# openai/gym

Hardware: AMD Instinct MI355X
Metric: env-steps/sec at num_envs=2^20, CartPole-v1 (higher is better)
Workload: dtype f64

## Files before the change

gym_amd/csrc/mxv_device.hpp:

```cpp
#pragma once
#include <hip/hip_runtime.h>
#include <stdint.h>

#include "../../include/mxv.h"
#include "../../include/mxv_diag.h"
#include "mxv_divide.hpp"

#define MXV_XFN __device__ inline
#define MXV_XCONST __device__ const
#define MXV_XCOLD __device__ __noinline__ inline
#include "mxv_exact.hpp"

namespace mxv {

struct EnvParams {
    double p[MXV_MAX_PARAMS];
};

enum { PM_BROADCAST = 0, PM_DEFAULT = 1, PM_PER_ENV = 2 };
template <int DEF>
struct Par {
    const EnvParams &P;
    const double *pe;
    int64_t n, e;
// ... 122 lines not shown
    return philox4x32_10_vkey(c, (uint32_t)seed, (uint32_t)(seed >> 32));
}

__device__ __forceinline__ uint32_t step_noise_word(uint64_t seed, uint64_t t) {
    U4 c;
    c.x = (uint32_t)t;
    c.y = (uint32_t)(t >> 32);
    c.z = 0;
    c.w = (kStreamStepNoise << 28);
    return philox4x32_10_vkey(c, (uint32_t)seed, (uint32_t)(seed >> 32)).x;
}

__device__ __forceinline__ double div_by_const(double x, double c, double rc) {
    const double q0 = x * rc;
    const double r = __fma_rn(-c, q0, x);
    return __fma_rn(r, rc, q0);
}
template <int DEF, bool FINITE = true>
__device__ __forceinline__ double div_par(double x, double c) {
    if constexpr (DEF == PM_DEFAULT && FINITE)
        return div_by_const(x, c, 1.0 / c);
    else if constexpr (DEF == PM_DEFAULT)
        return __builtin_amdgcn_div_fixup(div_by_const(x, c, 1.0 / c), c, x);
    else
        return x / c;
}

template <int ENV>
constexpr int fma3_for() {
    return ((ENV == MXV_PENDULUM || ENV == MXV_MOUNTAINCAR_CONT) ? 1 : 0) | ((ENV == MXV_ACROBOT || ENV == MXV_PENDULUM) ? 2 : 0);
}

template <int F3>
__device__ __forceinline__ double fma_coef(double a, double b, double k) {
    if constexpr ((F3 & 1) != 0) {
        double r;
        asm("v_fma_f64 %0, %1, %2, %3" : "=v"(r) : "v"(a), "v"(b), "v"(k));
        return r;
    } else {
        return __fma_rn(a, b, k);
    }
}

template <int F3 = 0>
__device__ __forceinline__ void sincos_kernel(double x, double *sn, double *cs) {
    const double z = x * x;
    double r = fma_coef<F3>(z, 1.58969099521155010221e-10, -2.50507602534068634195e-08);
    r = fma_coef<F3>(z, r, 2.75573137070700676789e-06);
    r = fma_coef<F3>(z, r, -1.98412698298579493134e-04);
    r = fma_coef<F3>(z, r, 8.33333333332248946124e-03);
    r = fma_coef<F3>(z, r, -1.66666666666666324348e-01);
    *sn = __fma_rn(x * z, r, x);
    double c = fma_coef<F3>(z, -1.13596475577881948265e-11, 2.08757232129817482790e-09);
    c = fma_coef<F3>(z, c, -2.75573143513906633035e-07);
    c = fma_coef<F3>(z, c, 2.48015872894767294178e-05);
    c = fma_coef<F3>(z, c, -1.38888888888741095749e-03);
    c = fma_coef<F3>(z, c, 4.16666666666666019037e-02);
    c = __fma_rn(z, c, -0.5);
    *cs = __fma_rn(z, c, 1.0);
}

template <int F3 = 0>
__device__ __forceinline__ void sincos_medium(double x, double *sn, double *cs) {
    const double k = rint(x * 6.36619772367581382433e-01);
    double r = __fma_rn(-k, 1.5707963267341256, x);
    r = __fma_rn(-k, 6.077100506303966e-11, r);
    r = __fma_rn(-k, 2.0222662487959506e-21, r);
    double s, c;
    sincos_kernel<F3>(r, &s, &c);
    const uint32_t q = (uint32_t)(int)k;
    const bool swap = (q & 1u) != 0u;
    const double ss = swap ? c : s, cc = swap ? s : c;
    if constexpr ((F3 & 2) != 0) {
        *sn = __hiloint2double((int)xor_masked(__double2hiint(ss), q << 30, 0x80000000u), __double2loint(ss));
        *cs = __hiloint2double((int)xor_masked(__double2hiint(cc), (q + 1u) << 30, 0x80000000u), __double2loint(cc));
    } else {
        *sn = __hiloint2double(__double2hiint(ss) ^ (int)((q & 2u) << 30), __double2loint(ss));
        *cs = __hiloint2double(__double2hiint(cc) ^ (int)(((q + 1u) & 2u) << 30), __double2loint(cc));
    }
}
template <bool GUARD = true, int F3 = 0>
__device__ __forceinline__ void mx_sincos(double x, double *sn, double *cs) {
    if constexpr (!GUARD) {
        sincos_medium<F3>(x, sn, cs);
    } else if (fabs(x) < 256.0) {
        sincos_medium<F3>(x, sn, cs);
        if (x == 0.0) *sn = x;
    } else {
        sincos(x, sn, cs);
    }
}
template <bool GUARD = true, int F3 = 0>
__device__ __forceinline__ double mx_cos(double x) {
    double s, c;
    mx_sincos<GUARD, F3>(x, &s, &c);
    return c;
}
template <bool GUARD = true, int F3 = 0>
__device__ __forceinline__ double mx_sin(double x) {
    double s, c;
    mx_sincos<GUARD, F3>(x, &s, &c);
    return s;
}

__device__ __forceinline__ void sincos_small_or_general(double x, double *sn, double *cs) {
    if (fabs(x) <= 0.78539816339744830962) {
        sincos_kernel(x, sn, cs);
        if (x == 0.0) *sn = x;
    } else {
        mx_sincos(x, sn, cs);
    }
}

__device__ __forceinline__ double nan_through(double x, double r) {
    const bool nan = x != x;
    return __hiloint2double(nan ? __double2hiint(x) : __double2hiint(r), nan ? __double2loint(x) : __double2loint(r));
}
__device__ __forceinline__ double clamp_range(double x, double lo, double hi) {
    return nan_through(x, __builtin_fmin(__builtin_fmax(x, lo), hi));
}
__device__ __forceinline__ float clamp_range(float x, float lo, float hi) {
    float r;
    asm("v_maximum3_f32 %0, %1, %2, %2" : "=v"(r) : "v"(x), "v"(lo));
    asm("v_minimum3_f32 %0, %1, %2, %2" : "=v"(r) : "v"(r), "v"(hi));
    return r;
}
__device__ __forceinline__ double clamp_range_hi_first(double x, double lo, double hi) {
    return nan_through(x, __builtin_fmax(__builtin_fmin(x, hi), lo));
}
__device__ __forceinline__ float clamp_range_hi_first(float x, float lo, float hi) {
    float r;
    asm("v_minimum3_f32 %0, %1, %2, %2" : "=v"(r) : "v"(x), "v"(hi));
    asm("v_maximum3_f32 %0, %1, %2, %2" : "=v"(r) : "v"(r), "v"(lo));
    return r;
}

__device__ __forceinline__ double fmod_const(double a, double b, double inv_b) {
    const double aa = fabs(a);
    if (!(aa < 1048576.0 * b)) return fmod(a, b);
    const double q = trunc(aa * inv_b);
    double r = __fma_rn(-q, b, aa);
    if (r < 0.0) r += b;
    else if (r >= b) r -= b;
    return copysign(r, a);
}

template <int ENV>
struct Env;

template <>
struct Env<MXV_CARTPOLE> {
    static constexpr int S = 4, O = 4, NA = 2;
    static constexpr int AUX = 0;
    template <bool GUARD = true>
    __device__ __forceinline__ static void prime(const double *s, double *aux) {}
    template <int DEF, bool SAFE = true, int EPL = 0>
    __device__ __forceinline__ static bool step(const Par<DEF> &P, double *s, double *, bool, int ai, float, double &reward,
                                                float *obs) {
        const double gravity = P.get(0, 9.8), masspole = P.get(2, 0.1), total_mass = P.get(3, 0.1 + 1.0);
        const double length = P.get(4, 0.5), polemass_length = P.get(5, 0.1 * 0.5), force_mag = P.get(6, 10.0);
        const double tau = P.get(7, 0.02), theta_thr = P.get(8, 12 * 2 * kPi / 360), x_thr = P.get(9, 2.4);
        const bool semi_implicit = P.get(10, 0.0) != 0.0;
        double x = s[0], x_dot = s[1], theta = s[2], theta_dot = s[3];
        const double force = (ai == 1) ? force_mag : -force_mag;
        double sintheta, costheta;
        if constexpr (DEF == PM_DEFAULT && !SAFE)
            sincos_kernel<((fma3_for<MXV_CARTPOLE>() & 1) || EPL == 1) ? 1 : 0>(theta, &sintheta, &costheta);
        else
            sincos_small_or_general(theta, &sintheta, &costheta);
        const double temp = div_par<DEF, !SAFE>(force + polemass_length * (theta_dot * theta_dot) * sintheta, total_mass);
        const double ta_num = gravity * sintheta - costheta * temp;
        const double ta_den = length * (4.0 / 3.0 - div_par<DEF, !SAFE>(masspole * (costheta * costheta), total_mass));
        double thetaacc;
        if constexpr (DEF == PM_DEFAULT && !SAFE)
            thetaacc = div_with_rcp(ta_num, ta_den, refined_rcp(ta_den));
        else
            thetaacc = ta_num / ta_den;
        const double xacc = temp - div_par<DEF, !SAFE>(polemass_length * thetaacc * costheta, total_mass);
        if (!semi_implicit) {
            x = x + tau * x_dot;
            x_dot = x_dot + tau * xacc;
            theta = theta + tau * theta_dot;
            theta_dot = theta_dot + tau * thetaacc;
        } else {
            x_dot = x_dot + tau * xacc;
            x = x + tau * x_dot;
            theta_dot = theta_dot + tau * thetaacc;
            theta = theta + tau * theta_dot;
        }
        s[0] = x; s[1] = x_dot; s[2] = theta; s[3] = theta_dot;
        reward = 1.0;
        obs[0] = (float)x; obs[1] = (float)x_dot; obs[2] = (float)theta; obs[3] = (float)theta_dot;
        return (x < -x_thr) || (x > x_thr) || (theta < -theta_thr) || (theta > theta_thr);
    }
    template <bool GUARD = true>
    __device__ __forceinline__ static void observe(const double *s, float *obs, double * = nullptr) {
        obs[0] = (float)s[0]; obs[1] = (float)s[1]; obs[2] = (float)s[2]; obs[3] = (float)s[3];
    }
    __device__ __forceinline__ static void reset(U4 w, double b0, double b1, double *s) {
        s[0] = b0 + (b1 - b0) * u01(w.x);
        s[1] = b0 + (b1 - b0) * u01(w.y);
        s[2] = b0 + (b1 - b0) * u01(w.z);
        s[3] = b0 + (b1 - b0) * u01(w.w);
    }
};

#ifndef MXV_PENDULUM_GLIBC_POWF
#define MXV_PENDULUM_GLIBC_POWF 0
#endif
static __device__ const uint64_t kExp2fTab[32] = {
    0x3ff0000000000000ull, 0x3fefd9b0d3158574ull, 0x3fefb5586cf9890full, 0x3fef9301d0125b51ull,
    0x3fef72b83c7d517bull, 0x3fef54873168b9aaull, 0x3fef387a6e756238ull, 0x3fef1e9df51fdee1ull,
    0x3fef06fe0a31b715ull, 0x3feef1a7373aa9cbull, 0x3feedea64c123422ull, 0x3feece086061892dull,
    0x3feebfdad5362a27ull, 0x3feeb42b569d4f82ull, 0x3feeab07dd485429ull, 0x3feea47eb03a5585ull,
    0x3feea09e667f3bcdull, 0x3fee9f75e8ec5f74ull, 0x3feea11473eb0187ull, 0x3feea589994cce13ull,
    0x3feeace5422aa0dbull, 0x3feeb737b0cdc5e5ull, 0x3feec49182a3f090ull, 0x3feed503b23e255dull,
    0x3feee89f995ad3adull, 0x3feeff76f2fb5e47ull, 0x3fef199bdd85529cull, 0x3fef3720dcef9069ull,
    0x3fef5818dcfba487ull, 0x3fef7c97337b9b5full, 0x3fefa4afa2a490daull, 0x3fefd0765b6e4540ull,
};
static __device__ const double kPowfLog2Tab[16][2] = {
    {0x1.661ec79f8f3bep+0, -0x1.efec65b963019p-2}, {0x1.571ed4aaf883dp+0, -0x1.b0b6832d4fca4p-2},
    {0x1.49539f0f010b0p+0, -0x1.7418b0a1fb77bp-2}, {0x1.3c995b0b80385p+0, -0x1.39de91a6dcf7bp-2},
    {0x1.30d190c8864a5p+0, -0x1.01d9bf3f2b631p-2}, {0x1.25e227b0b8ea0p+0, -0x1.97c1d1b3b7af0p-3},
    {0x1.1bb4a4a1a343fp+0, -0x1.2f9e393af3c9fp-3}, {0x1.12358f08ae5bap+0, -0x1.960cbbf788d5cp-4},
    {0x1.0953f419900a7p+0, -0x1.a6f9db6475fcep-5}, {0x1.0000000000000p+0, 0x0.0p+0},
    {0x1.e608cfd9a47acp-1, 0x1.338ca9f24f53dp-4},  {0x1.ca4b31f026aa0p-1, 0x1.476a9543891bap-3},
    {0x1.b2036576afce6p-1, 0x1.e840b4ac4e4d2p-3},  {0x1.9c2d163a1aa2dp-1, 0x1.40645f0c6651cp-2},
    {0x1.886e6037841edp-1, 0x1.88e9c2c1b9ff8p-2},  {0x1.767dcf5534862p-1, 0x1.ce0a44eb17bccp-2},
};
__device__ __forceinline__ float glibc_powf_square(float x) {
    uint32_t ix = __float_as_uint(x) & 0x7fffffffu;
    if (ix - 0x00800000u >= 0x7f800000u - 0x00800000u) {
        if (ix == 0u || ix >= 0x7f800000u) return x * x;
        ix = __float_as_uint(x * 0x1p23f) & 0x7fffffffu;
        ix -= 23u << 23;
    }
    const uint32_t tmp = ix - 0x3f330000u;
    const uint32_t i = (tmp >> 19) & 15u;
    const uint32_t top = tmp & 0xff800000u;
    const double k = (double)((int32_t)top >> 23);
    const double z = (double)__uint_as_float(ix - top);
    const double invc = kPowfLog2Tab[i][0], logc = kPowfLog2Tab[i][1];
    const double r = z * invc - 1.0;
    const double y0 = logc + k;
    const double r2 = r * r;
    double y = 0x1.27616c9496e0bp-2 * r + -0x1.71969a075c67ap-2;
    const double p = 0x1.ec70a6ca7baddp-2 * r + -0x1.7154748bef6c8p-1;
    const double r4 = r2 * r2;
    double q = 0x1.71547652ab82bp+0 * r + y0;
    q = p * r2 + q;
    y = y * r4 + q;
    const double ylogx = 2.0 * y;
    if (ylogx <= -150.0) return 0.0f;
    if (ylogx > 0x1.fffffffd1d571p+6) return __uint_as_float(0x7f800000u);
    double kd = ylogx + 0x1.8p+47;
    const uint64_t ki = (uint64_t)__double_as_longlong(kd);
    kd -= 0x1.8p+47;
    const double rr = ylogx - kd;
    uint64_t t = kExp2fTab[ki & 31u];
    t += ki << 47;
    const double sc = __longlong_as_double((long long)t);
    const double zz = 0x1.c6af84b912394p-5 * rr + 0x1.ebfce50fac4f3p-3;
    const double rr2 = rr * rr;
    double yy = 0x1.62e42ff0c52d6p-1 * rr + 1.0;
    yy = zz * rr2 + yy;
    yy = yy * sc;
    return (float)yy;
}

__device__ __forceinline__ double np_remainder(double a, double b) {
    double mod = fmod_const(a, b, 1.0 / b);
    if (b == 0.0) return mod;
    if (mod != 0.0) {
        if ((b < 0) != (mod < 0)) mod += b;
    } else {
        mod = copysign(0.0, b);
    }
    return mod;
}
__device__ __forceinline__ double np_remainder_bounded(double a, double b) {
    const double aa = fabs(a);
    const double q = trunc(aa * (1.0 / b));
    double r = __fma_rn(-q, b, aa);
    const double up = r + b, down = r - b;
    r = (r < 0.0) ? up : ((r >= b) ? down : r);
    double mod = copysign(r, a);
    const double lifted = mod + b;
    mod = (mod < 0.0) ? lifted : mod;
    return (mod == 0.0) ? 0.0 : mod;
}

template <>
struct Env<MXV_PENDULUM> {
    static constexpr int S = 2, O = 3, NA = 0;
    static constexpr int AUX = 1;
    template <bool GUARD = true>
    __device__ __forceinline__ static void prime(const double *s, double *aux) { aux[0] = mx_sin<GUARD, fma3_for<MXV_PENDULUM>()>(s[0]); }
    template <bool GUARD = true, int F3 = fma3_for<MXV_PENDULUM>()>
    __device__ __forceinline__ static void observe(const double *s, float *obs, double *aux) {
        double sn, cs;
        mx_sincos<GUARD, F3>(s[0], &sn, &cs);
        obs[0] = (float)cs; obs[1] = (float)sn; obs[2] = (float)s[1];
        aux[0] = sn;
    }
    template <int DEF, bool SAFE = true, int EPL = 0>
    __device__ __forceinline__ static bool step(const Par<DEF> &P, double *s, double *aux, bool, int, float a0,
// ... 296 lines not shown
```

gym_amd/csrc/mxv_kernels.hip:

```cpp
#include <cstdlib>
#include <type_traits>

#include "mxv_host.hpp"
#include "mxv_kernels.hpp"

namespace mxv {

namespace {

__device__ __forceinline__ void raise_error(int32_t *err, int32_t bit) { *reinterpret_cast<volatile int32_t *>(err) = bit; }

typedef float f32x4_t __attribute__((ext_vector_type(4)));
typedef float f32x2_t __attribute__((ext_vector_type(2)));
typedef int i32x4_t __attribute__((ext_vector_type(4)));
typedef int i32x2_t __attribute__((ext_vector_type(2)));
template <bool NT, typename T>
__device__ __forceinline__ void st(T *p, T v) {
    if constexpr (NT) __builtin_nontemporal_store(v, p);
    else *p = v;
}
__device__ __forceinline__ int32_t load_elapsed(const void *p, int32_t el16, int64_t e) {
    return el16 ? (int32_t) static_cast<const uint16_t *>(p)[e] : static_cast<const int32_t *>(p)[e];
}
template <bool NT = false>
// ... 261 lines not shown

        float obs[E][O];
        double rew[E];
        bool term[E], trunc[E], pend[E];
#pragma unroll
        for (int j = 0; j < E; ++j) {
            term[j] = EV::template step<DEF>(P.at(valid[j] ? env_of(j) : 0), s[j], aux[j], el[j] == 0, ai[j], af[j], rew[j], obs[j]);
            el[j] += 1;
            trunc[j] = (a.max_steps > 0) && (el[j] >= a.max_steps);
            pend[j] = autoreset && (term[j] || trunc[j]);
        }
        if (a.ep_acc != nullptr) {
#pragma unroll
            for (int j = 0; j < E; ++j) {
                er[j] = (float)((double)er[j] + rew[j]);
                if (valid[j] && (term[j] || trunc[j])) {
                    if (a.ep_return_out) a.ep_return_out[so + env_of(j)] = er[j];
                    if (a.ep_length_out) a.ep_length_out[so + env_of(j)] = el[j];
                    er[j] = 0.0f;
                }
            }
        }

        while (true) {
            int jsel = -1;
#pragma unroll
            for (int j = E - 1; j >= 0; --j)
                if (pend[j]) jsel = j;
            if (!__any(jsel >= 0)) break;
            if (jsel >= 0) {
                const int64_t e = tile0 + (int64_t)jsel * kBlock + tid;
                bool v = false;
                uint32_t k_reset = 0;
                float cur[O];
#pragma unroll
                for (int j = 0; j < E; ++j)
                    if (j == jsel) {
                        v = valid[j];
                        k_reset = ep[j];
#pragma unroll
                        for (int k = 0; k < O; ++k) cur[k] = obs[j][k];
                    }
                if (a.final_obs != nullptr && v) store_obs<O>(a.final_obs, so + e, cur);
                if constexpr (LAZY_EP) {
                    k_reset = landed(a.episodes[v ? e : 0]);
                    if (v) a.episodes[e] = k_reset + 1;
                }
                const uint64_t seed = a.seeds ? landed(a.seeds[v ? e : 0]) : a.base_seed + a.env0 + (uint64_t)e;
                const U4 w = episode_reset_words(seed, k_reset);
                double ns[S], naux[AUXN];
                float nobs[O];
                EV::reset(w, a.b0, a.b1, ns);
                EV::observe(ns, nobs, naux);
#pragma unroll
                for (int j = 0; j < E; ++j)
                    if (j == jsel) {
#pragma unroll
                        for (int k = 0; k < EV::AUX; ++k) aux[j][k] = naux[k];
#pragma unroll
                        for (int k = 0; k < S; ++k) s[j][k] = ns[k];
#pragma unroll
                        for (int k = 0; k < O; ++k) obs[j][k] = nobs[k];
                        el[j] = 0;
                        if constexpr (!LAZY_EP) ep[j] += 1;
                        pend[j] = false;
                    }
            }
        }

#pragma unroll
        for (int j = 0; j < E; ++j) {
            if (!valid[j]) continue;
            const int64_t e = so + env_of(j);
            store_obs<O, NT>(a.obs, e, obs[j]);
            if (a.reward != nullptr) {
                if (a.flags & MXV_FLAG_REWARD_F32)
                    st<NT>(static_cast<float *>(a.reward) + e, (float)rew[j]);
                else
                    st<NT>(static_cast<double *>(a.reward) + e, rew[j]);
            }
            if (a.terminated != nullptr) st<NT>(a.terminated + e, (uint8_t)(term[j] ? 1 : 0));
            if (a.truncated != nullptr) st<NT>(a.truncated + e, (uint8_t)(trunc[j] ? 1 : 0));
        }
        if constexpr (ENV == MXV_CARTPOLE) {
            if (a.beyond != nullptr) {
#pragma unroll
                for (int j = 0; j < E; ++j)
                    if (valid[j] && term[j]) {
                        uint8_t *mark = a.beyond + env_of(j);
                        if (landed((uint32_t)*mark) == 0u) {
                            *mark = 1;
                        } else if (a.reward != nullptr) {
                            if (a.flags & MXV_FLAG_REWARD_F32)
                                static_cast<float *>(a.reward)[so + env_of(j)] = 0.0f;
                            else
                                static_cast<double *>(a.reward)[so + env_of(j)] = 0.0;
                        }
                    }
            }
        }
    }

#pragma unroll
    for (int j = 0; j < E; ++j) {
        if (!valid[j]) continue;
        const int64_t e = env_of(j);
        if constexpr (HILO) {
            int32_t l[S];
            bool esc = false;
#pragma unroll
            for (int k = 0; k < S; ++k) {
                l[k] = hilo_encode_fast(s[j][k]);
                esc = esc || l[k] == kHiloEscape;
            }
            if (__builtin_expect(__any(esc), 0)) {
#pragma unroll
                for (int k = 0; k < S; ++k)
                    if (l[k] == kHiloEscape) a.state[(int64_t)k * n + e] = s[j][k];
            }
            store_lo<S, NT>(a.lo, e, l);
        } else {
#pragma unroll
            for (int k = 0; k < S; ++k) st<NT>(a.state + (int64_t)k * n + e, s[j][k]);
        }
        store_elapsed<NT>(a.elapsed, a.elapsed16, e, el[j]);
        if (ep[j] != ep_in[j]) a.episodes[e] = ep[j];
        if (a.ep_acc) a.ep_acc[e] = er[j];
    }
    if constexpr (CLOCK) {
        if (tid == 0) {
            const uint32_t ticket = atomicAdd(a.clock_ticket, 1u);
            if (ticket == gridDim.x - 1) {
                *a.clock_ticket = 0u;
                *a.clock_out = t0 - a.t + (uint64_t)a.K;
            }
        }
    }
}

constexpr int kWave = 64;
constexpr int kSimds = 1024;

template <int S, int O, int AUX>
struct alignas(16) ResetEntry {
    double s[S];
    double x[AUX];
    float o[O];
};
template <int S, int O>
struct alignas(16) ResetEntry<S, O, 0> {
    double s[S];
    float o[O];
};

template <int ENV, bool DEF, bool SAFE>
constexpr int rollout_min_waves() {
    return (!DEF || (ENV == MXV_CARTPOLE && SAFE)) ? 1 : 4;
}

template <int CTRL>
__device__ __forceinline__ double stat_dpp(double v) {
    const int lo = __builtin_amdgcn_update_dpp(0, __double2loint(v), CTRL, 0xF, 0xF, true);
    const int hi = __builtin_amdgcn_update_dpp(0, __double2hiint(v), CTRL, 0xF, 0xF, true);
    return __hiloint2double(hi, lo);
}
__device__ __forceinline__ double stat_xor4(double v) {
    const int lo = __builtin_amdgcn_ds_swizzle(__double2loint(v), 0x101F), hi = __builtin_amdgcn_ds_swizzle(__double2hiint(v), 0x101F);
    return __hiloint2double(hi, lo);
}
template <int CTRL, int N>
__device__ __forceinline__ void stat_halve(double (&v)[N], bool bit) {
#pragma unroll
    for (int p = 0; p < N / 2; ++p) {
        const double lo = v[2 * p], hi = v[2 * p + 1];
        v[p] = (bit ? hi : lo) + stat_dpp<CTRL>(bit ? lo : hi);
    }
}
template <int V>
__device__ __forceinline__ double wave_sums(double (&v)[V], uint32_t lane) {
    static_assert(V == 4 || V == 8, "batches of 4 or 8 values");
    stat_halve<0xB1, V>(v, (lane & 1u) != 0);
    if constexpr (V == 8) {
        double w[4] = {v[0], v[1], v[2], v[3]};
        stat_halve<0x4E, 4>(w, (lane & 2u) != 0);
        double u[2] = {w[0], w[1]};
        stat_halve<0x128, 2>(u, (lane & 8u) != 0);
        v[0] = u[0];
    } else {
        double w[2] = {v[0], v[1]};
        stat_halve<0x4E, 2>(w, (lane & 2u) != 0);
        v[0] = w[0] + stat_dpp<0x128>(w[0]);
    }
    double x = v[0];
    x += stat_xor4(x);
    {
        const unsigned lo = (unsigned)__double2loint(x), hi = (unsigned)__double2hiint(x);
        const auto a = __builtin_amdgcn_permlane16_swap(lo, lo, false, false), b = __builtin_amdgcn_permlane16_swap(hi, hi, false, false);
        x = __hiloint2double((int)b[0], (int)a[0]) + __hiloint2double((int)b[1], (int)a[1]);
    }
    {
        const unsigned lo = (unsigned)__double2loint(x), hi = (unsigned)__double2hiint(x);
        const auto a = __builtin_amdgcn_permlane32_swap(lo, lo, false, false), b = __builtin_amdgcn_permlane32_swap(hi, hi, false, false);
        x = __hiloint2double((int)b[0], (int)a[0]) + __hiloint2double((int)b[1], (int)a[1]);
    }
    return x;
}
template <int V>
__device__ __forceinline__ void wave_sums_store(double (&v)[V], uint32_t lane, double *dst, int count) {
    const double x = wave_sums<V>(v, lane);
    const uint32_t idx = V == 8 ? ((lane & 3u) | ((lane >> 1) & 4u)) : (lane & 3u);
    const bool holder = V == 8 ? (lane & 0x34u) == 0 : (lane & 0x3Cu) == 0;
    if (holder && (int)idx < count) dst[idx] = x;
}

template <int ENV, int E>
struct RolloutLds {
    static constexpr int TILE = E * kWave;
    static constexpr int H = kWave / (TILE / 4);
    using Entry = ResetEntry<Env<ENV>::S, Env<ENV>::O, Env<ENV>::AUX>;
    uint32_t act[H * TILE];
    Entry res[TILE];
};

template <int ENV, bool DEF, int E, bool SAFE, int OUT, bool TAPE = false, int STATS = 0>
__device__ __forceinline__ void rollout_body_v3(const StepArgs &a, const unsigned bid, const unsigned nblk, RolloutLds<ENV, E> &lds) {
    using EV = Env<ENV>;
    constexpr int S = EV::S, O = EV::O, NA = EV::NA;
    constexpr int TILE = E * kWave;
    constexpr int NACT = TILE / 4;
    constexpr int H = kWave / NACT;
    constexpr int SH = action_unit_shift<ENV>();
    constexpr int PERIOD = kRolloutPassPeriod;
    static_assert(NACT <= kWave && (PERIOD & (PERIOD - 1)) == 0 && PERIOD >= E, "E <= 4; pass period a power of two >= E");
    constexpr int AUXN = EV::AUX > 0 ? EV::AUX : 1;
    using Entry = ResetEntry<S, O, EV::AUX>;
    uint32_t *const lds_act = lds.act;
    Entry *const lds_res = lds.res;

    const int lane = threadIdx.x;
    const uint32_t tile = xcd_contiguous_tile(bid, nblk);
    const int64_t tile0 = (int64_t)tile * TILE;
    const int64_t n = a.n;
    const Par<DEF> P(a.P);
    const uint64_t t0 = a.t + (a.t_dev ? *a.t_dev : 0);
    constexpr bool FULL = OUT != 0;
    const bool act_i32 = FULL ? (OUT == 2) : ((a.flags & MXV_FLAG_ACTION_I32) != 0);
    const bool rew_f32 = FULL ? (OUT == 2) : ((a.flags & MXV_FLAG_REWARD_F32) != 0);
    const bool ep_on = !FULL && a.ep_acc != nullptr;
    const uint64_t group0 = (a.env0 + (uint64_t)tile0) >> 2;

    double s[E][S], aux[E][AUXN];
    int32_t el[E];
    uint32_t ep[E];
    bool valid[E];
    uint32_t le[E];
#pragma unroll
    for (int j = 0; j < E; ++j) {
        const int64_t e = tile0 + j * kWave + lane;
        valid[j] = e < n;
        le[j] = (uint32_t)(valid[j] ? e : 0);
#pragma unroll
        for (int k = 0; k < S; ++k) s[j][k] = a.state[(int64_t)k * n + le[j]];
        el[j] = load_elapsed(a.elapsed, a.elapsed16, le[j]);
        ep[j] = a.episodes[le[j]];
        EV::template prime<SAFE>(s[j], aux[j]);
    }
    float er[E];
#pragma unroll
    for (int j = 0; j < E; ++j) er[j] = ep_on ? a.ep_acc[le[j]] : 0.0f;
    float *p_epr = FULL ? nullptr : a.ep_return_out;
    int32_t *p_epl = FULL ? nullptr : a.ep_length_out;

    const uint64_t u0 = t0 >> SH;
    auto draw_units = [&](uint64_t q) {
        const U4 w = philox4x32_10(action_unit_counter<ENV>(u0 + q + (uint64_t)(lane / NACT), group0 + (uint64_t)(lane % NACT)),
                                   (uint32_t)a.action_seed, (uint32_t)(a.action_seed >> 32));
        reinterpret_cast<uint4 *>(lds_act)[lane] = make_uint4(w.x, w.y, w.z, w.w);
        __builtin_amdgcn_fence(__ATOMIC_RELEASE, "wavefront");
    };
    uint32_t word[E];
    if constexpr (!TAPE) {
        draw_units(0);
        __builtin_amdgcn_fence(__ATOMIC_ACQUIRE, "wavefront");
#pragma unroll
        for (int j = 0; j < E; ++j) word[j] = lds_act[j * kWave + lane];
    }
    const uint32_t tape_b = NA > 0 ? (act_i32 ? 4u : 8u) : 4u;
    const char *const p_tape = reinterpret_cast<const char *>(a.actions);
    struct TapeRegs {
        int64_t i[E];
        float f[E];
    } tape_even, tape_odd;
    auto load_tape = [&](int step, TapeRegs &r) {
        const char *base = p_tape + (int64_t)min(step, a.K - 1) * a.act_slice * (int64_t)tape_b;
#pragma unroll
        for (int j = 0; j < E; ++j) {
            const char *q = base + le[j] * tape_b;
            if constexpr (NA > 0)
                r.i[j] = act_i32 ? (int64_t) * reinterpret_cast<const int32_t *>(q) : *reinterpret_cast<const int64_t *>(q);
            else
                r.f[j] = *reinterpret_cast<const float *>(q);
        }
    };
    bool bad[E];
#pragma unroll
    for (int j = 0; j < E; ++j) bad[j] = false;
    if constexpr (TAPE) {
        load_tape(0, tape_even);
        load_tape(1, tape_odd);
    }

    bool need[E];
    auto fill_entries = [&](int j) {
        if (need[j]) {
            const uint64_t seed = a.seeds ? landed(a.seeds[le[j]]) : a.base_seed + a.env0 + (uint64_t)le[j];
            const U4 w = episode_reset_words(seed, ep[j]);
            Entry r;
            EV::reset(w, a.b0, a.b1, r.s);
            if constexpr (EV::AUX > 0) {
                EV::template observe<false>(r.s, r.o, r.x);
            } else {
                double none[1];
                EV::template observe<false>(r.s, r.o, none);
            }
            lds_res[j * kWave + lane] = r;
        }
        need[j] = false;
    };
#pragma unroll
    for (int j = 0; j < E; ++j) {
        need[j] = valid[j];
        fill_entries(j);
    }

    char *p_obs = reinterpret_cast<char *>(a.obs);
    char *p_rew = reinterpret_cast<char *>(a.reward);
    char *p_act = reinterpret_cast<char *>(a.actions_out);
    char *p_term = reinterpret_cast<char *>(a.terminated);
    char *p_trunc = reinterpret_cast<char *>(a.truncated);
    char *p_fin = FULL ? nullptr : reinterpret_cast<char *>(a.final_obs);
    [[maybe_unused]] double *p_part = (STATS & 1) ? a.obs_part + (int64_t)tile * (2 * O) : nullptr;
    [[maybe_unused]] double *p_rpart = (STATS & 2) ? a.ret_part + (int64_t)tile * 2 : nullptr;
    [[maybe_unused]] double ret[E], ret_s = 0.0, ret_q = 0.0;
#pragma unroll
    for (int j = 0; j < E; ++j) ret[j] = ((STATS & 2) && valid[j]) ? a.ret_state[le[j]] : 0.0;
    const uint32_t rew_b = rew_f32 ? 4u : 8u;
    const uint32_t act_b = (NA > 0 && !act_i32) ? 8u : 4u;
    uint32_t lo[E];
    const int64_t slice = a.slice;
#pragma unroll
    for (int j = 0; j < E; ++j) lo[j] = (uint32_t)(j * kWave + lane);
    p_obs += tile0 * (int64_t)(O * sizeof(float));
    if (p_rew) p_rew += tile0 * (int64_t)rew_b;
    if (p_act) p_act += tile0 * (int64_t)act_b;
    if (p_term) p_term += tile0;
    if (p_trunc) p_trunc += tile0;
    if (p_fin) p_fin += tile0 * (int64_t)(O * sizeof(float));
    if (p_epr) p_epr += tile0;
    if (p_epl) p_epl += tile0;

    settle_entry_loads();
    auto one_step = [&](const int step, auto allv_tag, TapeRegs &tape) __attribute__((always_inline)) {
        constexpr bool ALLV = decltype(allv_tag)::value;
        const uint64_t t = t0 + (uint64_t)step;

        int ai[E];
        float af[E];
        if constexpr (TAPE) {
#pragma unroll
            for (int j = 0; j < E; ++j) {
                if constexpr (NA > 0) {
                    const int64_t v = tape.i[j];
                    const bool oob = v < 0 || v >= NA;
                    if ((ALLV || valid[j]) && oob && !bad[j]) {
                        raise_error(a.err, 1);
                        bad[j] = true;
                    }
                    ai[j] = oob ? 0 : (int)v;
                    af[j] = 0.0f;
                } else {
                    ai[j] = 0;
                    af[j] = tape.f[j];
                }
            }
            load_tape(step + 2, tape);
        } else {
#pragma unroll
            for (int j = 0; j < E; ++j) action_from_word<ENV, DEF>(P, word[j], t, ai[j], af[j]);
        }
        if (TAPE ? (!FULL && p_act != nullptr) : (FULL || p_act != nullptr)) {
#pragma unroll
            for (int j = 0; j < E; ++j) {
                if (!ALLV && !valid[j]) continue;
                char *q = p_act + pin32(lo[j] * act_b);
                if constexpr (NA > 0) {
                    if (act_i32)
                        *reinterpret_cast<int32_t *>(q) = ai[j];
                    else
                        *reinterpret_cast<int64_t *>(q) = (int64_t)ai[j];
                } else {
                    *reinterpret_cast<float *>(q) = af[j];
                }
            }
        }

        float obs[E][O];
        double rew[E];
        bool term[E], trunc[E], pend[E];
#pragma unroll
        for (int j = 0; j < E; ++j) {
            term[j] = EV::template step<DEF, SAFE, E>(P, s[j], aux[j], el[j] == 0, ai[j], af[j], rew[j], obs[j]);
            el[j] += 1;
            trunc[j] = (a.max_steps > 0) && (el[j] >= a.max_steps);
            pend[j] = (ALLV || valid[j]) && (term[j] || trunc[j]);
        }
        if constexpr ((STATS & 2) != 0) {
            ret_s = ret_q = 0.0;
#pragma unroll
            for (int j = 0; j < E; ++j) {
                const double r = rew_f32 ? (double)(float)rew[j] : rew[j];
                ret[j] = ret[j] * a.ret_gamma + r;
                if (ALLV || valid[j]) {
                    ret_s += ret[j];
                    ret_q = __fma_rn(ret[j], ret[j], ret_q);
                }
                if (term[j] || trunc[j]) ret[j] = 0.0;
            }
        }
        if (ep_on) {
#pragma unroll
            for (int j = 0; j < E; ++j) {
                er[j] = (float)((double)er[j] + rew[j]);
                if (pend[j]) {
                    if (p_epr) *reinterpret_cast<float *>(reinterpret_cast<char *>(p_epr) + pin32(lo[j] * 4u)) = er[j];
                    if (p_epl) *reinterpret_cast<int32_t *>(reinterpret_cast<char *>(p_epl) + pin32(lo[j] * 4u)) = el[j];
                    er[j] = 0.0f;
                }
            }
        }
#pragma unroll
        for (int j = 0; j < E; ++j) {
            if (!ALLV && !valid[j]) continue;
            if (FULL || p_rew != nullptr) {
                char *q = p_rew + pin32(lo[j] * rew_b);
                if (rew_f32)
                    *reinterpret_cast<float *>(q) = (float)rew[j];
                else
                    *reinterpret_cast<double *>(q) = rew[j];
            }
            if (FULL || p_term != nullptr) *reinterpret_cast<uint8_t *>(p_term + pin32(lo[j])) = term[j] ? 1 : 0;
            if (FULL || p_trunc != nullptr) *reinterpret_cast<uint8_t *>(p_trunc + pin32(lo[j])) = trunc[j] ? 1 : 0;
            if (!FULL && pend[j] && p_fin != nullptr) store_obs_at<O>(p_fin, pin32(lo[j] * (uint32_t)(O * sizeof(float))), obs[j]);
        }

#pragma unroll
        for (int j = 0; j < E; ++j) {
            if (__any(pend[j])) {
                if (__any(pend[j] && need[j])) fill_entries(j);
                if (pend[j]) {
                    const Entry r = lds_res[j * kWave + lane];
#pragma unroll
                    for (int k = 0; k < S; ++k) s[j][k] = r.s[k];
                    if constexpr (EV::AUX > 0) {
#pragma unroll
                        for (int k = 0; k < EV::AUX; ++k) aux[j][k] = r.x[k];
                    }
#pragma unroll
                    for (int k = 0; k < O; ++k) obs[j][k] = r.o[k];
                    el[j] = 0;
                    ep[j] += 1;
                    need[j] = true;
                }
            }
        }

        if (!TAPE && step + 1 < a.K) {
            const uint64_t q0 = (t >> SH) - u0, q1 = ((t + 1) >> SH) - u0;
            if (SH == 0 || q1 != q0) {
                if (q1 % H == 0) draw_units(q1);
                __builtin_amdgcn_fence(__ATOMIC_ACQUIRE, "wavefront");
#pragma unroll
                for (int j = 0; j < E; ++j) word[j] = lds_act[(uint32_t)(q1 % H) * TILE + j * kWave + lane];
            }
        }
#pragma unroll
        for (int j = 0; j < E; ++j)
            if (ALLV || valid[j]) store_obs_at<O>(p_obs, pin32(lo[j] * (uint32_t)(O * sizeof(float))), obs[j]);
        if constexpr ((STATS & 1) != 0) {
            double sm[O], sq[O];
#pragma unroll
            for (int k = 0; k < O; ++k) sm[k] = sq[k] = 0.0;
#pragma unroll
            for (int j = 0; j < E; ++j) {
#pragma unroll
                for (int k = 0; k < O; ++k) {
                    const double x = (ALLV || valid[j]) ? (double)obs[j][k] : 0.0;
                    sm[k] += x;
                    sq[k] = __fma_rn(x, x, sq[k]);
                }
            }
            if constexpr (2 * O <= 8) {
                constexpr int V = 2 * O <= 4 ? 4 : 8;
                double v[V];
#pragma unroll
                for (int k = 0; k < V; ++k) v[k] = 0.0;
#pragma unroll
                for (int k = 0; k < O; ++k) {
                    v[k] = sm[k];
                    v[O + k] = sq[k];
                }
                wave_sums_store<V>(v, (uint32_t)lane, p_part, 2 * O);
            } else {
                static_assert(O <= 8, "two batches of at most 8 values");
                double v[8], w[8];
#pragma unroll
                for (int k = 0; k < 8; ++k) v[k] = w[k] = 0.0;
#pragma unroll
                for (int k = 0; k < O; ++k) {
                    v[k] = sm[k];
                    w[k] = sq[k];
                }
                wave_sums_store<8>(v, (uint32_t)lane, p_part, O);
                wave_sums_store<8>(w, (uint32_t)lane, p_part + O, O);
            }
            p_part += (int64_t)nblk * (2 * O);
        }
        if constexpr ((STATS & 2) != 0) {
            double v[4] = {ret_s, ret_q, 0.0, 0.0};
            wave_sums_store<4>(v, (uint32_t)lane, p_rpart, 2);
            p_rpart += (int64_t)nblk * 2;
        }
        if (step + 1 == a.K && a.snap_obs != nullptr) {
#pragma unroll
            for (int j = 0; j < E; ++j) {
                if (!ALLV && !valid[j]) continue;
                store_obs<O>(a.snap_obs, le[j], obs[j]);
                if (a.snap_reward != nullptr) {
                    if (rew_f32)
                        static_cast<float *>(a.snap_reward)[le[j]] = (float)rew[j];
                    else
                        static_cast<double *>(a.snap_reward)[le[j]] = rew[j];
                }
                if (a.snap_terminated != nullptr) a.snap_terminated[le[j]] = term[j] ? 1 : 0;
                if (a.snap_truncated != nullptr) a.snap_truncated[le[j]] = trunc[j] ? 1 : 0;
            }
        }

#pragma unroll
        for (int j = 0; j < E; ++j)
            if ((step & (PERIOD - 1)) == j * (PERIOD / E) && __any(need[j])) fill_entries(j);

        p_obs += slice * (int64_t)(O * sizeof(float));
        if (FULL || p_rew != nullptr) p_rew += slice * (int64_t)rew_b;
        if (TAPE ? (!FULL && p_act != nullptr) : (FULL || p_act != nullptr)) p_act += slice * (int64_t)act_b;
        if (FULL || p_term != nullptr) p_term += slice;
        if (FULL || p_trunc != nullptr) p_trunc += slice;
        if (!FULL && p_fin != nullptr) p_fin += slice * (int64_t)(O * sizeof(float));
        if (!FULL && p_epr != nullptr) p_epr += slice;
        if (!FULL && p_epl != nullptr) p_epl += slice;
    };
    if constexpr (TAPE) {
        auto run_pairs = [&](auto allv_tag) __attribute__((always_inline)) {
            int step = 0;
            for (; step + 1 < a.K; step += 2) {
                one_step(step, allv_tag, tape_even);
                one_step(step + 1, allv_tag, tape_odd);
            }
            if (step < a.K) one_step(step, allv_tag, tape_even);
        };
        bool allv = true;
#pragma unroll
        for (int j = 0; j < E; ++j) allv = allv && __all(valid[j]);
        if (allv)
            run_pairs(std::true_type{});
        else
            run_pairs(std::false_type{});
    } else {
        for (int step = 0; step < a.K; ++step) one_step(step, std::false_type{}, tape_even);
    }

#pragma unroll
    for (int j = 0; j < E; ++j) {
        if (!valid[j] || bad[j]) continue;
#pragma unroll
        for (int k = 0; k < S; ++k) a.state[(int64_t)k * n + le[j]] = s[j][k];
        store_elapsed(a.elapsed, a.elapsed16, le[j], el[j]);
        a.episodes[le[j]] = ep[j];
        if (ep_on) a.ep_acc[le[j]] = er[j];
        if constexpr ((STATS & 2) != 0) a.ret_state[le[j]] = ret[j];
    }
}


template <int ENV, bool DEF, bool SAFE>
constexpr int rollout_max_waves() {
    return rollout_min_waves<ENV, DEF, SAFE>() == 1 ? 8 : rollout_min_waves<ENV, DEF, SAFE>();
}

template <int ENV, bool DEF, int E, bool SAFE, int OUT = 0, bool TAPE = false, int STATS = 0>
__global__ void __launch_bounds__(kWave)
    __attribute__((amdgpu_waves_per_eu(rollout_min_waves<ENV, DEF, SAFE>(), rollout_max_waves<ENV, DEF, SAFE>())))
    rollout_kernel_v3(const StepArgs a) {
    __shared__ RolloutLds<ENV, E> lds;
    rollout_body_v3<ENV, DEF, E, SAFE, OUT, TAPE, STATS>(a, blockIdx.x, gridDim.x, lds);
}

union MixedLds {
    RolloutLds<MXV_CARTPOLE, 1> cartpole;
    RolloutLds<MXV_PENDULUM, 1> pendulum;
    RolloutLds<MXV_ACROBOT, 1> acrobot;
    RolloutLds<MXV_MOUNTAINCAR, 1> mountaincar;
    RolloutLds<MXV_MOUNTAINCAR_CONT, 1> mountaincar_cont;
    __device__ MixedLds() {}
};

__global__ void __launch_bounds__(kWave) mixed_rollout_kernel(const MixedArgs m) {
    __shared__ MixedLds lds;
    unsigned sidx = 0;
#pragma unroll
    for (int i = 1; i < MXV_MAX_MIXED; ++i)
        if (i < m.count && blockIdx.x >= m.first_block[i]) sidx = (unsigned)i;
    const StepArgs &a = m.seg[sidx];
    const unsigned bid = blockIdx.x - m.first_block[sidx], nblk = m.first_block[sidx + 1] - m.first_block[sidx];
    switch (m.kind[sidx]) {
        case MXV_CARTPOLE:
            rollout_body_v3<MXV_CARTPOLE, true, 1, true, 0>(a, bid, nblk, lds.cartpole);
            break;
        case MXV_PENDULUM: rollout_body_v3<MXV_PENDULUM, true, 1, true, 0>(a, bid, nblk, lds.pendulum); break;
        case MXV_ACROBOT: rollout_body_v3<MXV_ACROBOT, true, 1, true, 0>(a, bid, nblk, lds.acrobot); break;
        case MXV_MOUNTAINCAR: rollout_body_v3<MXV_MOUNTAINCAR, true, 1, true, 0>(a, bid, nblk, lds.mountaincar); break;
        default: rollout_body_v3<MXV_MOUNTAINCAR_CONT, true, 1, true, 0>(a, bid, nblk, lds.mountaincar_cont); break;
    }
}

template <int ENV>
__global__ void __launch_bounds__(kBlock) reset_kernel(const ResetArgs a) {
    using EV = Env<ENV>;
    constexpr int S = EV::S, O = EV::O;
    const int64_t e = (int64_t)blockIdx.x * kBlock + threadIdx.x;
    if (e >= a.n) return;
    if (a.mask != nullptr && a.mask[e] == 0) return;
    const uint64_t seed = a.seeds ? landed(a.seeds[e]) : a.base_seed + a.env0 + (uint64_t)e;
    const uint32_t k = a.episodes[e];
    a.episodes[e] = k + 1u;
    const U4 w = episode_reset_words(seed, k);
    double s[S];
    EV::reset(w, a.b0, a.b1, s);
#pragma unroll
    for (int k = 0; k < S; ++k) a.state[(int64_t)k * a.n + e] = s[k];
    store_elapsed(a.elapsed, a.elapsed16, e, 0);
    if (a.ep_acc != nullptr) a.ep_acc[e] = 0.0f;
    if (a.beyond != nullptr) a.beyond[e] = 0;
    if (a.obs != nullptr) {
        float o[O];
        double aux_unused[EV::AUX > 0 ? EV::AUX : 1];
        EV::observe(s, o, aux_unused);
        store_obs<O>(a.obs, e, o);
    }
}

template <int ENV, int DEF>
__global__ void __launch_bounds__(kBlock) sample_kernel(const SampleArgs a) {
    constexpr int NA = Env<ENV>::NA;
    const int64_t c = (int64_t)blockIdx.x * kBlock + threadIdx.x;
    if (c * 4 >= a.n) return;
    const Par<DEF> P(a.P, a.params_pe, a.n);
    const uint64_t t = a.t + (a.t_dev ? *a.t_dev : 0);
    const U4 w = env_action_words<ENV>(a.action_seed, t, (a.env0 >> 2) + (uint64_t)c);
    const uint32_t ws[4] = {w.x, w.y, w.z, w.w};
#pragma unroll
    for (int q = 0; q < 4; ++q) {
        const int64_t e = c * 4 + q;
        if (e >= a.n) break;
        int ai;
        float af;
        action_from_word<ENV, DEF>(P.at(e), ws[q], t, ai, af);
        if constexpr (NA > 0) {
            if (a.flags & MXV_FLAG_ACTION_I32)
                static_cast<int32_t *>(a.actions_out)[e] = ai;
            else
                static_cast<int64_t *>(a.actions_out)[e] = ai;
        } else {
            static_cast<float *>(a.actions_out)[e] = af;
        }
    }
}

__global__ void set_word_kernel(uint64_t *dst, uint64_t value) { *dst = value; }
__global__ void add_word_kernel(uint64_t *dst, uint64_t delta) { *dst += delta; }

constexpr int kCompactChunk = 4096, kCompactIters = kCompactChunk / kBlock, kCompactWaves = kBlock / kWave;

__device__ __forceinline__ bool compact_done(const CompactArgs &a, int64_t e) {
    return e < a.n && (a.terminated[e] | a.truncated[e]) != 0;
}

__global__ void __launch_bounds__(kBlock) final_count_kernel(const CompactArgs a) {
    __shared__ int32_t part[kCompactWaves];
    const int64_t e0 = (int64_t)blockIdx.x * kCompactChunk + threadIdx.x;
    int32_t c = 0;
#pragma unroll 4
    for (int i = 0; i < kCompactIters; ++i) c += (int32_t)__popcll(__ballot(compact_done(a, e0 + (int64_t)i * kBlock)));
    if (threadIdx.x % kWave == 0) part[threadIdx.x / kWave] = c;
// ... 394 lines not shown
```

Before: 184.8 billion.

## Slim CartPole reset LDS entries and track reset-need as wave ballot masks

For environments whose observation equals the state and that carry no auxiliary data (CartPole), the LDS reset entry drops the float observation copy. Observations are instead recomputed from state after the reset merge each step. The per-lane bool 'need' flags become 64-bit wave ballot masks, so the any-reductions become scalar mask tests. This is meant to cut LDS footprint and traffic and vector compare work, at the cost of an extra observe call on every step for every lane.

```diff
diff --git a/gym_amd/csrc/mxv_device.hpp b/gym_amd/csrc/mxv_device.hpp
--- a/gym_amd/csrc/mxv_device.hpp
+++ b/gym_amd/csrc/mxv_device.hpp
@@ -298,6 +298,7 @@
 struct Env<MXV_CARTPOLE> {
     static constexpr int S = 4, O = 4, NA = 2;
     static constexpr int AUX = 0;
+    static constexpr bool OBS_IS_STATE = true;
     template <bool GUARD = true>
     __device__ __forceinline__ static void prime(const double *s, double *aux) {}
     template <int DEF, bool SAFE = true, int EPL = 0>
diff --git a/gym_amd/csrc/mxv_kernels.hip b/gym_amd/csrc/mxv_kernels.hip
--- a/gym_amd/csrc/mxv_kernels.hip
+++ b/gym_amd/csrc/mxv_kernels.hip
@@ -437,6 +437,18 @@
     double s[S];
     float o[O];
 };
+template <int S>
+struct alignas(16) ResetEntry<S, 0, 0> {
+    double s[S];
+};
+template <class EV, class = void>
+struct obs_is_state : std::false_type {};
+template <class EV>
+struct obs_is_state<EV, std::enable_if_t<EV::OBS_IS_STATE>> : std::true_type {};
+template <int ENV>
+constexpr int entry_obs() {
+    return (obs_is_state<Env<ENV>>::value && Env<ENV>::AUX == 0) ? 0 : Env<ENV>::O;
+}
 
 template <int ENV, bool DEF, bool SAFE>
 constexpr int rollout_min_waves() {
@@ -502,7 +514,7 @@
 struct RolloutLds {
     static constexpr int TILE = E * kWave;
     static constexpr int H = kWave / (TILE / 4);
-    using Entry = ResetEntry<Env<ENV>::S, Env<ENV>::O, Env<ENV>::AUX>;
+    using Entry = ResetEntry<Env<ENV>::S, entry_obs<ENV>(), Env<ENV>::AUX>;
     uint32_t act[H * TILE];
     Entry res[TILE];
 };
@@ -518,7 +530,8 @@
     constexpr int PERIOD = kRolloutPassPeriod;
     static_assert(NACT <= kWave && (PERIOD & (PERIOD - 1)) == 0 && PERIOD >= E, "E <= 4; pass period a power of two >= E");
     constexpr int AUXN = EV::AUX > 0 ? EV::AUX : 1;
-    using Entry = ResetEntry<S, O, EV::AUX>;
+    constexpr bool SLIM = entry_obs<ENV>() == 0;
+    using Entry = typename RolloutLds<ENV, E>::Entry;
     uint32_t *const lds_act = lds.act;
     Entry *const lds_res = lds.res;
 
@@ -595,26 +608,26 @@
         load_tape(1, tape_odd);
     }
 
-    bool need[E];
+    uint64_t need[E];
     auto fill_entries = [&](int j) {
-        if (need[j]) {
+        if (__builtin_amdgcn_inverse_ballot_w64(need[j])) {
             const uint64_t seed = a.seeds ? landed(a.seeds[le[j]]) : a.base_seed + a.env0 + (uint64_t)le[j];
             const U4 w = episode_reset_words(seed, ep[j]);
             Entry r;
             EV::reset(w, a.b0, a.b1, r.s);
             if constexpr (EV::AUX > 0) {
                 EV::template observe<false>(r.s, r.o, r.x);
-            } else {
+            } else if constexpr (!SLIM) {
                 double none[1];
                 EV::template observe<false>(r.s, r.o, none);
             }
             lds_res[j * kWave + lane] = r;
         }
-        need[j] = false;
+        need[j] = 0;
     };
 #pragma unroll
     for (int j = 0; j < E; ++j) {
-        need[j] = valid[j];
+        need[j] = __builtin_amdgcn_ballot_w64(valid[j]);
         fill_entries(j);
     }
 
@@ -740,8 +753,9 @@
 
 #pragma unroll
         for (int j = 0; j < E; ++j) {
-            if (__any(pend[j])) {
-                if (__any(pend[j] && need[j])) fill_entries(j);
+            const uint64_t done = __builtin_amdgcn_ballot_w64(pend[j]);
+            if (done != 0) {
+                if ((done & need[j]) != 0) fill_entries(j);
                 if (pend[j]) {
                     const Entry r = lds_res[j * kWave + lane];
 #pragma unroll
@@ -750,13 +764,19 @@
 #pragma unroll
                         for (int k = 0; k < EV::AUX; ++k) aux[j][k] = r.x[k];
                     }
-#pragma unroll
-                    for (int k = 0; k < O; ++k) obs[j][k] = r.o[k];
+                    if constexpr (!SLIM) {
+#pragma unroll
+                        for (int k = 0; k < O; ++k) obs[j][k] = r.o[k];
+                    }
                     el[j] = 0;
                     ep[j] += 1;
-                    need[j] = true;
                 }
-            }
+                need[j] |= done;
+            }
+        }
+        if constexpr (SLIM) {
+#pragma unroll
+            for (int j = 0; j < E; ++j) EV::template observe<false>(s[j], obs[j]);
         }
 
         if (!TAPE && step + 1 < a.K) {
@@ -833,7 +853,7 @@
 
 #pragma unroll
         for (int j = 0; j < E; ++j)
-            if ((step & (PERIOD - 1)) == j * (PERIOD / E) && __any(need[j])) fill_entries(j);
+            if ((step & (PERIOD - 1)) == j * (PERIOD / E) && need[j] != 0) fill_entries(j);
 
         p_obs += slice * (int64_t)(O * sizeof(float));
         if (FULL || p_rew != nullptr) p_rew += slice * (int64_t)rew_b;
```

Result: no change. 185.0 billion (median of 2 runs) (+0.1%).
